# Ghostish/Open3DSOT

Hardware: NVIDIA H100
Metric: template-search pairs/sec, BAT-Car fwd+bwd (higher is better)
Workload: dtype f32

## Files before the change

open3dsot_b200/csrc/pwmlp_tc.cu:

```cuda
#include "common.cuh"
#include "lift.cuh"
#include "tc_ptx.cuh"
#include "../../include/o3d_b200.h"

namespace {

struct TcAct {
    const float* x; int ld; const float* scale; const float* shift; int relu;
    struct Coef { float4 s, t; bool on; };
    template <int R> struct Batch { float4 v[R]; };
    __device__ __forceinline__ Coef prep(int k, int K) const {
        Coef c;
        c.on = k < K;
        c.s = make_float4(1.f, 1.f, 1.f, 1.f);
        c.t = make_float4(0.f, 0.f, 0.f, 0.f);
        if (c.on && scale) { c.s = ld4g(scale + k); c.t = ld4g(shift + k); }
        return c;
    }
    template <int R>
    __device__ __forceinline__ void fetch(Batch<R>& b, int p0, int stride, int P, int k, int K) const {
        const int kk = k < K ? k : 0;
#pragma unroll
        for (int i = 0; i < R; ++i) {
            const int p = p0 + i * stride;
            b.v[i] = ld4g(x + (size_t)(p < P ? p : P - 1) * ld + kk);
        }
    }
    template <int R>
    __device__ __forceinline__ float4 finish(const Batch<R>& b, const Coef& c, int i, int p, int P) const {
        float4 v = b.v[i];
        if (!(c.on && p < P)) return make_float4(0.f, 0.f, 0.f, 0.f);
        if (scale) { v.x = fmaf(v.x, c.s.x, c.t.x); v.y = fmaf(v.y, c.s.y, c.t.y); v.z = fmaf(v.z, c.s.z, c.t.z); v.w = fmaf(v.w, c.s.w, c.t.w); }
        if (relu) { v.x = fmaxf(v.x, 0.f); v.y = fmaxf(v.y, 0.f); v.z = fmaxf(v.z, 0.f); v.w = fmaxf(v.w, 0.f); }
        return v;
    }
    __device__ __forceinline__ void prefetch_rows(int p0, int rows, int P) const {
        if (p0 < P) o3d_prefetch_l2(x + (size_t)p0 * ld, (size_t)min(rows, P - p0) * ld * sizeof(float));
    }
};

struct TcLift {
    LiftView lv; const float* scale; const float* shift; int relu;
    int la;
    struct Coef { float4 s, t, u0, u1, u2, u3; bool on; };
    template <int R> struct Batch { float4 v[R]; float4 sv[R]; int nrow[R]; int tag; };
    __device__ __forceinline__ Coef prep(int k, int K) const {
        Coef c;
        c.on = k < K;
        c.s = make_float4(1.f, 1.f, 1.f, 1.f);
        c.t = c.u0 = c.u1 = c.u2 = c.u3 = make_float4(0.f, 0.f, 0.f, 0.f);
        if (c.on && scale) { c.s = ld4g(scale + k); c.t = ld4g(shift + k); }
        if (c.on && lv.u) { c.u0 = ld4g(lv.u + k); c.u1 = ld4g(lv.u + lv.ldz + k); c.u2 = ld4g(lv.u + 2 * lv.ldz + k); c.u3 = ld4g(lv.u + 3 * lv.ldz + k); }
        return c;
    }
    template <int R>
    __device__ __forceinline__ void fetch(Batch<R>& b, int p0, int stride, int P, int k, int K) const {
        const int kk = k < K ? k : 0;
        if (lv.z) {
            int row[R];
            if (b.tag == p0 + 1) {
#pragma unroll
                for (int i = 0; i < R; ++i) row[i] = b.nrow[i];
            } else if (R == 4 && stride == 1 && (p0 & 3) == 0 && p0 + 3 < P) {
                const int4 r4 = __ldg(reinterpret_cast<const int4*>(lv.gidx + p0));
                row[0] = r4.x; row[R > 1 ? 1 : 0] = r4.y; row[R > 2 ? 2 : 0] = r4.z; row[R > 3 ? 3 : 0] = r4.w;
            } else {
#pragma unroll
                for (int i = 0; i < R; ++i) {
                    const int p = p0 + i * stride;
                    row[i] = __ldg(lv.gidx + (p < P ? p : P - 1));
                }
            }
#pragma unroll
            for (int i = 0; i < R; ++i) b.v[i] = ld4g(lv.z + (size_t)row[i] * lv.ldz + kk);
            if (la == 0) {
#pragma unroll
                for (int i = 0; i < R; ++i) b.nrow[i] = row[i];
                b.tag = p0 + 1;
            } else {
                const int pn = p0 + la;
#pragma unroll
                for (int i = 0; i < R; ++i) {
                    const int p = pn + i * stride;
                    b.nrow[i] = __ldg(lv.gidx + (p < P ? p : P - 1));
                }
                b.tag = pn + 1;
            }
        }
        if (lv.s) {
#pragma unroll
            for (int i = 0; i < R; ++i) {
                const int p = p0 + i * stride;
                b.sv[i] = ld4g(lv.s + (size_t)(p < P ? p : P - 1) * 4);
            }
        }
    }
    template <int R>
    __device__ __forceinline__ float4 finish(const Batch<R>& b, const Coef& c, int i, int p, int P) const {
        const float4 zero = make_float4(0.f, 0.f, 0.f, 0.f);
        if (!(c.on && p < P)) return zero;
        float4 v = lift_val4(lv.z ? b.v[i] : zero, lv.s ? b.sv[i] : zero, c.u0, c.u1, c.u2, c.u3);
        if (scale) { v.x = fmaf(v.x, c.s.x, c.t.x); v.y = fmaf(v.y, c.s.y, c.t.y); v.z = fmaf(v.z, c.s.z, c.t.z); v.w = fmaf(v.w, c.s.w, c.t.w); }
        if (relu) { v.x = fmaxf(v.x, 0.f); v.y = fmaxf(v.y, 0.f); v.z = fmaxf(v.z, 0.f); v.w = fmaxf(v.w, 0.f); }
        return v;
    }
    __device__ __forceinline__ void prefetch_rows(int p0, int rows, int P) const {
        if (p0 >= P) return;
        const size_t n = (size_t)min(rows, P - p0);
        if (lv.z) o3d_prefetch_l2(lv.gidx + p0, n * sizeof(int32_t));
        if (lv.s) o3d_prefetch_l2(lv.s + (size_t)p0 * 4, n * 16);
    }
};

struct TcDy {
    const float* g; int ldg; const float* y; int ldy; const float* a; const float* b; const float* cc;
    const float* dpool; const int32_t* sel; int S; int ldp;
    int sh;
    struct Coef { float4 a, b, c; bool on; };
    template <int R> struct Batch { float4 g[R]; float4 y[R]; bool shared; };
    __device__ __forceinline__ Coef prep(int k, int K) const {
        Coef c;
        c.on = k < K;
        c.a = make_float4(1.f, 1.f, 1.f, 1.f);
        c.b = c.c = make_float4(0.f, 0.f, 0.f, 0.f);
        if (c.on && a) { c.a = ld4g(a + k); c.b = ld4g(b + k); c.c = ld4g(cc + k); }
        return c;
    }
    template <int R>
    __device__ __forceinline__ void fetch(Batch<R>& bt, int p0, int stride, int P, int k, int K) const {
        const int kk = k < K ? k : 0;
        bt.shared = false;
        if (dpool) {
            const int pf = p0 < P ? p0 : P - 1;
            const int pe = p0 + (R - 1) * stride;
            const int pl = pe < P ? pe : P - 1;
            if (R >= 2 && (pf >> sh) == (pl >> sh)) {
                bt.shared = true;
                const size_t go = (size_t)(pf >> sh) * ldp + kk;
                bt.g[0] = ld4g(dpool + go);
                const int4 sl = __ldg(reinterpret_cast<const int4*>(sel + go));
                bt.g[R >= 2 ? 1 : 0] = make_float4(__int_as_float(sl.x), __int_as_float(sl.y), __int_as_float(sl.z), __int_as_float(sl.w));
            } else {
#pragma unroll
                for (int i = 0; i < R; ++i) {
                    const int p = p0 + i * stride, pp = p < P ? p : P - 1;
                    const int s = pp & (S - 1);
                    const size_t go = (size_t)(pp >> sh) * ldp + kk;
                    const int4 sl = __ldg(reinterpret_cast<const int4*>(sel + go));
                    const float4 d = ld4g(dpool + go);
                    bt.g[i] = make_float4(sl.x == s ? d.x : 0.f, sl.y == s ? d.y : 0.f, sl.z == s ? d.z : 0.f, sl.w == s ? d.w : 0.f);
                }
            }
        } else {
#pragma unroll
            for (int i = 0; i < R; ++i) {
                const int p = p0 + i * stride;
                bt.g[i] = ld4g(g + (size_t)(p < P ? p : P - 1) * ldg + kk);
            }
        }
#pragma unroll
        for (int i = 0; i < R; ++i) {
            const int p = p0 + i * stride;
            bt.y[i] = a ? ld4g(y + (size_t)(p < P ? p : P - 1) * ldy + kk) : make_float4(0.f, 0.f, 0.f, 0.f);
        }
    }
    template <int R>
    __device__ __forceinline__ float4 finish(const Batch<R>& bt, const Coef& c, int i, int p, int P) const {
        if (!(c.on && p < P)) return make_float4(0.f, 0.f, 0.f, 0.f);
        float4 v = bt.g[i];
        if (bt.shared) {
            const int s = p & (S - 1);
            const float4 d = bt.g[0], sl = bt.g[R >= 2 ? 1 : 0];
            v = make_float4(__float_as_int(sl.x) == s ? d.x : 0.f, __float_as_int(sl.y) == s ? d.y : 0.f,
                            __float_as_int(sl.z) == s ? d.z : 0.f, __float_as_int(sl.w) == s ? d.w : 0.f);
        }
        if (a) {
            const float4 yy = bt.y[i];
            v.x = fmaf(c.a.x, v.x, fmaf(c.c.x, yy.x, c.b.x)); v.y = fmaf(c.a.y, v.y, fmaf(c.c.y, yy.y, c.b.y));
            v.z = fmaf(c.a.z, v.z, fmaf(c.c.z, yy.z, c.b.z)); v.w = fmaf(c.a.w, v.w, fmaf(c.c.w, yy.w, c.b.w));
        }
        return v;
    }
    __device__ __forceinline__ void prefetch_rows(int p0, int rows, int P) const {
        if (p0 >= P) return;
        const size_t n = (size_t)min(rows, P - p0);
        if (!dpool) o3d_prefetch_l2(g + (size_t)p0 * ldg, n * ldg * sizeof(float));
        if (a) o3d_prefetch_l2(y + (size_t)p0 * ldy, n * ldy * sizeof(float));
        if (dpool) {
            const int g0 = p0 >> sh, g1 = (p0 + (int)n - 1) >> sh;
            const size_t bytes = (size_t)(g1 - g0 + 1) * ldp * sizeof(float);
            o3d_prefetch_l2(dpool + (size_t)g0 * ldp, bytes);
            o3d_prefetch_l2(sel + (size_t)g0 * ldp, bytes);
        }
    }
};

template <class L> struct Bf16 : L {};
template <class L> struct is_bf16 { static constexpr bool value = false; };
template <class L> struct is_bf16<Bf16<L>> { static constexpr bool value = true; };

template <int LD>
struct TcFwdEpi {
    float* y; int ldy; const float* bias; double* sum; double* sumsq;
    int S, log2S; float* ymax; float* ymin; int32_t* arg; int ldp;
    float bv, mx, mn; int ax, an; double d1, d2;
    __device__ __forceinline__ void begin(int ch, int Nw) {
        d1 = d2 = 0.0;
        bv = (bias && ch < Nw) ? bias[ch] : 0.f;
        mx = -INFINITY; mn = INFINITY; ax = an = 0;
    }
    __device__ __forceinline__ void prefetch(int, int, int, int) {}
    __device__ __forceinline__ const int32_t* lift_gidx() const { return nullptr; }
    __device__ __forceinline__ const float* lift_s() const { return nullptr; }
    __device__ __forceinline__ void set_tile(const int32_t*, const float4*) {}
    __device__ __forceinline__ void group(const uint32_t (&r)[16], int ch, int Nw, int pbase, int P) {
        if (ch >= Nw) return;
        float s1 = 0.f, s2 = 0.f;
        const int smask = S - 1;
        float* yp = y ? y + (size_t)pbase * ldy + ch : nullptr;
        if (pbase + 16 <= P && (S == 0 || S >= 16)) {
            float v[16];
#pragma unroll
            for (int j = 0; j < 16; ++j) v[j] = __uint_as_float(r[j]) + bv;
            if (yp) {
                const size_t st = LD ? (size_t)LD : (size_t)ldy;
#pragma unroll
                for (int j = 0; j < 16; ++j) yp[j * st] = v[j];
            }
#pragma unroll
            for (int j = 0; j < 16; ++j) {
                s1 += v[j];
                s2 = fmaf(v[j], v[j], s2);
            }
            if (S > 0) {
                float gm = v[0], gn = v[0];
                int ga = 0, gb = 0;
#pragma unroll
                for (int j = 1; j < 16; ++j) {
                    if (v[j] > gm) { gm = v[j]; ga = j; }
                    if (v[j] < gn) { gn = v[j]; gb = j; }
                }
                const int s0 = pbase & smask;
                if (s0 == 0) { mx = gm; ax = ga; mn = gn; an = gb; }
                else {
                    if (gm > mx) { mx = gm; ax = s0 + ga; }
                    if (gn < mn) { mn = gn; an = s0 + gb; }
                }
                if (s0 + 16 == S) {
                    const size_t o = (size_t)(pbase >> log2S) * ldp + ch;
                    ymax[o] = mx; ymin[o] = mn; arg[o] = ax | (an << 16);
                }
            }
        } else {
#pragma unroll
            for (int j = 0; j < 16; ++j) {
                if (pbase + j >= P) break;
                const float v = __uint_as_float(r[j]) + bv;
                if (yp) yp[(size_t)j * ldy] = v;
                s1 += v;
                s2 = fmaf(v, v, s2);
                if (S > 0) {
                    const int s = (pbase + j) & smask;
                    if (s == 0) { mx = -INFINITY; mn = INFINITY; ax = an = 0; }
                    if (v > mx) { mx = v; ax = s; }
                    if (v < mn) { mn = v; an = s; }
                    if (s == smask) {
                        const size_t o = (size_t)((pbase + j) >> log2S) * ldp + ch;
                        ymax[o] = mx; ymin[o] = mn; arg[o] = ax | (an << 16);
                    }
                }
            }
        }
        d1 += (double)s1;
        d2 += (double)s2;
    }
// ... 181 lines not shown
                                             kb == 0);
                }
                wgmma_commit();
                wgmma_wait<0>();
                wgmma_fence_acc(acc);
                if (lane == 0) o3d_mbar_arrive(empty + stage);
                if (++stage == TC_STAGES) { stage = 0; phase ^= 1; }
            }
            asm volatile("bar.sync %0, 128;" ::"r"(2 + h) : "memory");
            stage_acc(acc, stg, TC_EPI_LD);
            asm volatile("bar.sync %0, 128;" ::"r"(2 + h) : "memory");
            const float* row = stg + tw * TC_EPI_LD;
#pragma unroll 1
            for (int cg = 0; cg < 4; ++cg) {
                uint32_t r[16];
#pragma unroll
                for (int j = 0; j < 4; ++j) {
                    const float4 v = *reinterpret_cast<const float4*>(row + cg * 16 + 4 * j);
                    r[4 * j] = __float_as_uint(v.x); r[4 * j + 1] = __float_as_uint(v.y);
                    r[4 * j + 2] = __float_as_uint(v.z); r[4 * j + 3] = __float_as_uint(v.w);
                }
                epi.group(r, ch, Nw, pb + cg * 16, P);
                if (cg + 1 < 4) epi.prefetch(ch, Nw, pb + (cg + 1) * 16, P);
            }
            buf ^= 1;
        }
        epi.end(ch, Nw);
    } else {
        const int pt = (warp - 8) * 32 + lane;
        const int chunk = pt & 7;
        const int row0 = (pt >> 3) * 4;
        int stage = 0, phase = 0;
        struct Cur { int t, kb, p0; };
        auto advance = [&](Cur& c) {
            if (++c.kb == nkb) {
                c.kb = 0;
                c.t += gridDim.x;
                if (c.t < n_ptiles) c.p0 = tile_of(c.t) * TC_N;
            }
        };
        using Batch4 = typename BLoad::template Batch<4>;
        auto issue = [&](Batch4& r, typename BLoad::Coef& cf, const Cur& c) {
            if (c.t >= n_ptiles) return;
            const int k = c.kb * TC_K + chunk * 4;
            cf = bl.prep(k, K);
            bl.fetch(r, c.p0 + row0, 1, P, k, K);
        };
        Cur c0{(int)blockIdx.x, 0, 0};
        if (c0.t < n_ptiles) c0.p0 = tile_of(c0.t) * TC_N;
        Batch4 r0{};
        typename BLoad::Coef f0 = bl.prep(chunk * 4, K);
        issue(r0, f0, c0);
        if (pt == 0 && c0.t < n_ptiles) bl.prefetch_rows(c0.p0, TC_N, P);
        while (c0.t < n_ptiles) {
            o3d_mbar_wait(empty + stage, phase ^ 1);
            if (pt == 0) {
                o3d_mbar_expect_tx(full + stage, WBYTES);
                o3d_bulk_g2s(smem + stage * TC_STAGE_BYTES, wtiles + ((size_t)mt0 * nkb + c0.kb) * WBYTES, WBYTES, full + stage);
                const int tn = c0.t + (int)gridDim.x;
                if (c0.kb == 0 && tn < n_ptiles) bl.prefetch_rows(tile_of(tn) * TC_N, TC_N, P);
            }
            uint8_t* xhi = smem + stage * TC_STAGE_BYTES + 2 * TILE_BYTES;
            uint8_t* xlo = xhi + TILE_BYTES;
#pragma unroll
            for (int i = 0; i < 4; ++i) {
                const float4 v = bl.finish(r0, f0, i, c0.p0 + row0 + i, P);
                if constexpr (BF) {
                    *reinterpret_cast<uint2*>(xhi + sw64(row0 + i, chunk >> 1) + (chunk & 1) * 8) = pack_bf16x4(v);
                } else {
                    const uint32_t off = sw128(row0 + i, chunk);
                    *reinterpret_cast<float4*>(xhi + off) = hi_part(v);
                    *reinterpret_cast<float4*>(xlo + off) = lo_part(v);
                }
            }
            o3d_fence_proxy_async();
            o3d_mbar_arrive(full + stage);
            if (++stage == TC_STAGES) { stage = 0; phase ^= 1; }
            advance(c0);
            issue(r0, f0, c0);
        }
    }
}

constexpr int WG_STAGES = 3;
constexpr int WG_AHEAD = 4;
constexpr int WG_THREADS = 512;
constexpr int WG_SMEM = WG_STAGES * 4 * TILE_BYTES + 1024 + 256;

template <class L>
__device__ __forceinline__ void store_transposed(const L& ld, const typename L::template Batch<4>& raw, const typename L::Coef& cf,
                                                 uint8_t* hi, int c_local, int p_first, int prow0, int pend) {
#pragma unroll
    for (int i = 0; i < 4; ++i) {
        const int pl = prow0 + 8 * i;
        const float4 v = ld.finish(raw, cf, i, p_first + pl, pend);
        const float e[4] = {v.x, v.y, v.z, v.w};
#pragma unroll
        for (int j = 0; j < 4; ++j) {
            const uint32_t off = sw128(c_local + j, pl >> 2) + (uint32_t)((pl & 3) * 4);
            const float h = hi1(e[j]);
            *reinterpret_cast<float*>(hi + off) = h;
            *reinterpret_cast<float*>(hi + TILE_BYTES + off) = e[j] - h;
        }
    }
}

template <class XB>
__global__ void __launch_bounds__(WG_THREADS, 1)
    pw_wgrad_tc_kernel(TcDy da, XB xb, int P, int M, int N, int chunk, float* __restrict__ part) {
    extern __shared__ uint8_t smem_raw[];
    uint8_t* smem = reinterpret_cast<uint8_t*>((reinterpret_cast<uintptr_t>(smem_raw) + 1023) & ~(uintptr_t)1023);
    uint64_t* full = reinterpret_cast<uint64_t*>(smem + WG_STAGES * 4 * TILE_BYTES);
    uint64_t* empty = full + WG_STAGES;

    const int warp = threadIdx.x >> 5, lane = threadIdx.x & 31;
    const int m0 = blockIdx.z * TC_M, n0 = blockIdx.y * TC_N;
    const int pbeg = blockIdx.x * chunk, pend = min(P, pbeg + chunk);
    const int nkb = pend > pbeg ? (pend - pbeg + TC_K - 1) / TC_K : 0;
    auto kpos = [&](int i) { return pbeg + i * TC_K; };

    if (threadIdx.x == 0) {
        for (int s = 0; s < WG_STAGES; ++s) {
            o3d_mbar_init(full + s, 256);
            o3d_mbar_init(empty + s, 8);
        }
        o3d_fence_mbar_init();
    }
    __syncthreads();

    if (warp < 8) {
        const int h = warp >> 2, w = warp & 3;
        float acc[64];
#pragma unroll
        for (int i = 0; i < 64; ++i) acc[i] = 0.f;
        int stage = 0, phase = 0;
        for (int kb = 0; kb < nkb; ++kb) {
            o3d_mbar_wait(full + stage, phase);
            const uint32_t sb = o3d_smem_u32(smem + stage * 4 * TILE_BYTES);
            const uint32_t ab = sb + h * (TILE_BYTES / 2);
            wgmma_fence_acc(acc);
            wgmma_fence();
            wgmma_3xtf32_kblock<128>(acc, make_desc(ab), make_desc(ab + TILE_BYTES), make_desc(sb + 2 * TILE_BYTES),
                                     make_desc(sb + 3 * TILE_BYTES), kb == 0);
            wgmma_commit();
            wgmma_wait<0>();
            wgmma_fence_acc(acc);
            if (lane == 0) o3d_mbar_arrive(empty + stage);
            if (++stage == WG_STAGES) { stage = 0; phase ^= 1; }
        }
        const int Mt = TC_M * (int)gridDim.z, Nt = TC_N * (int)gridDim.y;
        float* __restrict__ out = part + (size_t)blockIdx.x * Mt * Nt;
#pragma unroll
        for (int i = 0; i < 64; i += 4) {
#pragma unroll
            for (int rr = 0; rr < 2; ++rr) {
                const int m = m0 + h * 64 + 16 * w + (lane >> 2) + 8 * rr, n = n0 + 8 * (i >> 2) + 2 * (lane & 3);
                *reinterpret_cast<float2*>(out + (size_t)m * Nt + n) = make_float2(acc[i + 2 * rr], acc[i + 2 * rr + 1]);
            }
        }
    } else {
        const int pw = warp - 8;
        const int c4 = pw * 4 + (lane & 3), prow0 = lane >> 2;
        const bool pt0 = pw == 0 && lane == 0;
        TcDy::Batch<4> ra = {};
        typename XB::template Batch<4> rb = {};
        auto fetch = [&](int kb) {
            da.fetch(ra, kpos(kb) + prow0, 8, pend, m0 + c4 * 4, M);
            xb.fetch(rb, kpos(kb) + prow0, 8, pend, n0 + c4 * 4, N);
        };
        auto prefetch = [&](int kb) {
            if (pt0 && kb < nkb) {
                da.prefetch_rows(kpos(kb), TC_K, pend);
                xb.prefetch_rows(kpos(kb), TC_K, pend);
            }
        };
        int stage = 0, phase = 0;
        for (int kb = 0; kb < WG_AHEAD; ++kb) prefetch(kb);
        if (nkb > 0) fetch(0);
        for (int kb = 0; kb < nkb; ++kb) {
            prefetch(kb + WG_AHEAD);
            o3d_mbar_wait(empty + stage, phase ^ 1);
            uint8_t* sbase = smem + stage * 4 * TILE_BYTES;
            store_transposed(da, ra, da.prep(m0 + c4 * 4, M), sbase, c4 * 4, kpos(kb), prow0, pend);
            store_transposed(xb, rb, xb.prep(n0 + c4 * 4, N), sbase + 2 * TILE_BYTES, c4 * 4, kpos(kb), prow0, pend);
            o3d_fence_proxy_async();
            o3d_mbar_arrive(full + stage);
            if (kb + 1 < nkb) fetch(kb + 1);
            if (++stage == WG_STAGES) { stage = 0; phase ^= 1; }
        }
    }
}

__global__ void __launch_bounds__(256)
    wgrad_reduce_kernel(const float* __restrict__ part, int splits, int Mt, int Nt, int M, int N, float* __restrict__ dW,
                        int lddw) {
    const int sub = threadIdx.x & 7;
    const int n4 = (blockIdx.x * 32 + (threadIdx.x >> 3)) * 4, m = blockIdx.y;
    float4 acc = make_float4(0.f, 0.f, 0.f, 0.f);
    if (n4 < N && m < M) {
        const float* p = part + (size_t)m * Nt + n4;
        for (int s = sub; s < splits; s += 8) {
            const float4 v = __ldg(reinterpret_cast<const float4*>(p + (size_t)s * Mt * Nt));
            acc.x += v.x; acc.y += v.y; acc.z += v.z; acc.w += v.w;
        }
    }
#pragma unroll
    for (int o = 4; o >= 1; o >>= 1) {
        acc.x += __shfl_xor_sync(0xFFFFFFFFu, acc.x, o); acc.y += __shfl_xor_sync(0xFFFFFFFFu, acc.y, o);
        acc.z += __shfl_xor_sync(0xFFFFFFFFu, acc.z, o); acc.w += __shfl_xor_sync(0xFFFFFFFFu, acc.w, o);
    }
    if (sub == 0 && n4 < N && m < M) {
        float* o = dW + (size_t)m * lddw + n4;
        o[0] += acc.x;
        if (n4 + 1 < N) o[1] += acc.y;
        if (n4 + 2 < N) o[2] += acc.z;
        if (n4 + 3 < N) o[3] += acc.w;
    }
}

__global__ void w_pretile_kernel(const float* __restrict__ W, int ld, int rows, int K, int nkb, uint8_t* __restrict__ out) {
    const int m_tile = blockIdx.y, kb = blockIdx.x;
    uint8_t* dst = out + ((size_t)m_tile * nkb + kb) * (2 * TILE_BYTES);
    for (int id = threadIdx.x; id < TC_M * 8; id += blockDim.x) {
        const int r = id >> 3, c = id & 7;
        const int row = m_tile * TC_M + r, k = kb * TC_K + c * 4;
        float4 v = make_float4(0.f, 0.f, 0.f, 0.f);
        if (row < rows && k < K) v = *reinterpret_cast<const float4*>(W + (size_t)row * ld + k);
        const uint32_t off = sw128(r, c);
        *reinterpret_cast<float4*>(dst + off) = hi_part(v);
        *reinterpret_cast<float4*>(dst + TILE_BYTES + off) = lo_part(v);
    }
}

inline int ilog2_exact(int v) { int l = 0; while ((1 << l) < v) ++l; return l; }

template <class BLoad, class Epi>
int launch_tc(BLoad bl, const uint8_t* wtiles, int P, int K, int Nw, Epi epi, bool reverse, cudaStream_t st, const char* name) {
    auto kern = pw_tc_kernel<BLoad, Epi>;
    O3D_CUDA(cudaFuncSetAttribute(kern, cudaFuncAttributeMaxDynamicSharedMemorySize, TC_SMEM), name);
    const int gy = (Nw + TC_M - 1) / TC_M;
    const int nkb = (K + TC_K - 1) / TC_K;
    const int n_ptiles = (P + TC_N - 1) / TC_N;
    int gx = o3d_num_sms() / gy;
    if (gx < 1) gx = 1;
    if (gx > n_ptiles) gx = n_ptiles;
    kern<<<dim3(gx, gy), TC_THREADS, TC_SMEM, st>>>(bl, wtiles, P, K, Nw, nkb, epi, reverse);
    O3D_CHECK_LAUNCH(name);
    return O3D_OK;
}

template <int LD, class BLoad>
int launch_fwd(const BLoad& bl, const void* wtiles, const float* bias, int P, int K, int Nw, float* y, int ldy, double* sum,
               double* sumsq, int S, float* ymax, float* ymin, int32_t* arg, int ldp, bool reverse, cudaStream_t st) {
    TcFwdEpi<LD> ep{};
    ep.y = y; ep.ldy = ldy; ep.bias = bias; ep.sum = sum; ep.sumsq = sumsq;
    ep.S = S; ep.ymax = ymax; ep.ymin = ymin; ep.arg = arg; ep.ldp = ldp;
    ep.log2S = 0;
    while ((1 << ep.log2S) < S) ++ep.log2S;
    return launch_tc(bl, (const uint8_t*)wtiles, P, K, Nw, ep, reverse, st, "o3d_pw_fwd_tc");
}

template <int LD, bool LIFT = false>
int launch_dgrad(const TcDy& bl, const void* wtiles_t, int P, int Cout, int Cin, float* out, int ldo, const float* yprev,
                 int ldyp, const float* pscale, const float* pshift, int prelu, double* s1, double* s2y, cudaStream_t st,
                 const LiftView* lv = nullptr) {
    if constexpr (!LIFT) {
        if (lv) return launch_dgrad<LD, true>(bl, wtiles_t, P, Cout, Cin, out, ldo, yprev, ldyp, pscale, pshift, prelu, s1, s2y, st, lv);
    }
    TcDgradEpi<LD, LIFT> ep{};
    if (lv) ep.lv = *lv;
    ep.out = out; ep.ldo = ldo; ep.yprev = yprev; ep.ldyp = ldyp; ep.scale = pscale; ep.shift = pshift; ep.relu = prelu;
    ep.s1g = s1; ep.s2y = s2y;
// ... 17 lines not shown
    return O3D_OK;
}

int o3d_pw_fwd_tc_dir(const float* x, int ldx, const float* in_scale, const float* in_shift, int in_relu, const void* wtiles,
                      const float* bias, int P, int K, int N, float* y, int ldy, double* sum, double* sumsq, int S, float* ymax,
                      float* ymin, int32_t* arg, int ldp, void* stream, bool reverse, bool bf16) {
    O3D_REQUIRE(x && wtiles, O3D_ERR_ARG, "o3d_pw_fwd_tc: null pointer");
    O3D_REQUIRE(P >= 0 && K >= 4 && N >= 1 && (K & 3) == 0 && (ldx & 3) == 0, O3D_ERR_ARG, "o3d_pw_fwd_tc: bad sizes");
    O3D_REQUIRE(S == 0 || (P % S == 0 && 64 % S == 0 && ymax && ymin && arg), O3D_ERR_ARG,
                "o3d_pw_fwd_tc: pooling group size must divide 64 and P");
    if (P == 0) return O3D_OK;
    const int Nw = (N + 3) & ~3;
    TcAct bl{x, ldx, in_scale, in_shift, in_relu};
    cudaStream_t st = (cudaStream_t)stream;
    if (bf16) {
        Bf16<TcAct> bb{bl};
#define O3D_FWD_ARGS bb, wtiles, bias, P, K, Nw, y, ldy, sum, sumsq, S, ymax, ymin, arg, ldp, reverse, st
        if (ldy == 64) return launch_fwd<64>(O3D_FWD_ARGS);
        if (ldy == 128) return launch_fwd<128>(O3D_FWD_ARGS);
        if (ldy == 256) return launch_fwd<256>(O3D_FWD_ARGS);
        return launch_fwd<0>(O3D_FWD_ARGS);
#undef O3D_FWD_ARGS
    }
#define O3D_FWD_ARGS bl, wtiles, bias, P, K, Nw, y, ldy, sum, sumsq, S, ymax, ymin, arg, ldp, reverse, st
    if (ldy == 64) return launch_fwd<64>(O3D_FWD_ARGS);
    if (ldy == 128) return launch_fwd<128>(O3D_FWD_ARGS);
    if (ldy == 256) return launch_fwd<256>(O3D_FWD_ARGS);
    return launch_fwd<0>(O3D_FWD_ARGS);
#undef O3D_FWD_ARGS
}

extern "C" int o3d_pw_fwd_tc(const float* x, int ldx, const float* in_scale, const float* in_shift, int in_relu,
                             const void* wtiles, const float* bias, int P, int K, int N, float* y, int ldy, double* sum,
                             double* sumsq, int S, float* ymax, float* ymin, int32_t* arg, int ldp, void* stream) {
    return o3d_pw_fwd_tc_dir(x, ldx, in_scale, in_shift, in_relu, wtiles, bias, P, K, N, y, ldy, sum, sumsq, S, ymax, ymin, arg,
                             ldp, stream, false, false);
}

namespace {
int dgrad_tc_impl(const float* g, int ldg, const float* y, int ldy, const float* a, const float* b, const float* cc,
                  const float* dpool, const int32_t* sel, int S, int ldp, const void* wtiles_t, int P, int Cout, int Cin,
                  float* out, int ldo, const float* yprev, int ldyp, const float* pscale, const float* pshift, int prelu,
                  double* s1, double* s2y, void* stream, const LiftView* lv) {
    O3D_REQUIRE((g || dpool) && wtiles_t && out, O3D_ERR_ARG, "o3d_pw_dgrad_tc: null pointer");
    O3D_REQUIRE((Cout & 3) == 0 && (Cin & 3) == 0, O3D_ERR_ARG, "o3d_pw_dgrad_tc: channel counts must be multiples of 4");
    if (P == 0) return O3D_OK;
    TcDy bl{g, ldg, y, ldy, a, b, cc, dpool, sel, S > 0 ? S : 1, ldp, ilog2_exact(S > 0 ? S : 1)};
    cudaStream_t st = (cudaStream_t)stream;
    const int ld = (!yprev || ldyp == ldo) ? ldo : 0;
#define O3D_DG_ARGS bl, wtiles_t, P, Cout, Cin, out, ldo, yprev, ldyp, pscale, pshift, prelu, s1, s2y, st, lv
    if (ld == 64) return launch_dgrad<64>(O3D_DG_ARGS);
    if (ld == 128) return launch_dgrad<128>(O3D_DG_ARGS);
    if (ld == 256) return launch_dgrad<256>(O3D_DG_ARGS);
    return launch_dgrad<0>(O3D_DG_ARGS);
#undef O3D_DG_ARGS
}
}

extern "C" int o3d_pw_dgrad_tc(const float* g, int ldg, const float* y, int ldy, const float* a, const float* b,
                               const float* cc, const float* dpool, const int32_t* sel, int S, int ldp,
                               const void* wtiles_t, int P, int Cout, int Cin, float* out, int ldo, const float* yprev,
                               int ldyp, const float* pscale, const float* pshift, int prelu, double* s1, double* s2y,
                               void* stream) {
    return dgrad_tc_impl(g, ldg, y, ldy, a, b, cc, dpool, sel, S, ldp, wtiles_t, P, Cout, Cin, out, ldo, yprev, ldyp, pscale,
                         pshift, prelu, s1, s2y, stream, nullptr);
}

extern "C" int o3d_pw_dgrad_tc_lift(const float* g, int ldg, const float* y, int ldy, const float* a, const float* b,
                                    const float* cc, const float* dpool, const int32_t* sel, int S, int ldp,
                                    const void* wtiles_t, int P, int Cout, int Cin, float* out, int ldo,
                                    const o3d_lift_t* lf, const int32_t* gidx, const float* pscale, const float* pshift,
                                    int prelu, double* s1, double* s2y, void* stream) {
    O3D_REQUIRE(lf && (gidx || !lf->z) && (lf->z || lf->s) && lf->ldz == Cin, O3D_ERR_ARG, "o3d_pw_dgrad_tc_lift: lift descriptor");
    const LiftView lv{lf->z, lf->ldz, lf->z ? gidx : nullptr, lf->s, lf->u};
    return dgrad_tc_impl(g, ldg, y, ldy, a, b, cc, dpool, sel, S, ldp, wtiles_t, P, Cout, Cin, out, ldo, nullptr, 0, pscale,
                         pshift, prelu, s1, s2y, stream, &lv);
}

namespace {
template <class XB>
int launch_wgrad(const TcDy& da, const XB& xb, int P, int Cout, int Cin, float* dw, int lddw, float* part, long long part_floats,
                 cudaStream_t st) {
    auto kern = pw_wgrad_tc_kernel<XB>;
    O3D_CUDA(cudaFuncSetAttribute(kern, cudaFuncAttributeMaxDynamicSharedMemorySize, WG_SMEM), "o3d_pw_wgrad_tc2");
    const int mt = (Cout + TC_M - 1) / TC_M, nt = (Cin + TC_N - 1) / TC_N;
    const int Mt = mt * TC_M, Nt = nt * TC_N;
    int splits = o3d_num_sms() / (mt * nt);
    if (splits < 1) splits = 1;
    const long long cap = part_floats / ((long long)Mt * Nt);
    if (splits > cap) splits = (int)cap;
    const int by_size = (P + 127) / 128;
    if (splits > by_size) splits = by_size;
    O3D_REQUIRE(splits >= 1, O3D_ERR_ARG, "o3d_pw_wgrad_tc2: workspace too small");
    int chunk = (P + splits - 1) / splits;
    chunk = ((chunk + TC_K - 1) / TC_K) * TC_K;
    splits = (P + chunk - 1) / chunk;
    kern<<<dim3(splits, nt, mt), WG_THREADS, WG_SMEM, st>>>(da, xb, P, Cout, Cin, chunk, part);
    O3D_CHECK_LAUNCH("o3d_pw_wgrad_tc2");
    dim3 rg((Cin / 4 + 31) / 32, Cout);
    wgrad_reduce_kernel<<<rg, 256, 0, st>>>(part, splits, Mt, Nt, Cout, Cin, dw, lddw);
    O3D_CHECK_LAUNCH("o3d_pw_wgrad_tc2: reduce");
    return O3D_OK;
}
inline TcLift make_tclift(const o3d_lift_t* lf, const int32_t* gidx, const float* scale, const float* shift, int relu) {
    return TcLift{LiftView{lf->z, lf->ldz, lf->z ? gidx : nullptr, lf->s, lf->u}, scale, shift, relu, 0};
}
}

extern "C" long long o3d_pw_wgrad_tc2_workspace_floats(void) {
    return (long long)o3d_num_sms() * TC_M * TC_N;
}

extern "C" int o3d_pw_wgrad_tc2(const float* g, int ldg, const float* y, int ldy, const float* a, const float* b,
                                const float* cc, const float* dpool, const int32_t* sel, int S, int ldp, const float* x,
                                int ldx, const float* in_scale, const float* in_shift, int in_relu, int P, int Cout,
                                int Cin, float* dw, int lddw, float* part, long long part_floats, void* stream) {
    O3D_REQUIRE((g || dpool) && x && dw && part, O3D_ERR_ARG, "o3d_pw_wgrad_tc2: null pointer");
    O3D_REQUIRE((Cout & 3) == 0 && (Cin & 3) == 0 && (ldx & 3) == 0 && (lddw & 3) == 0, O3D_ERR_ARG,
                "o3d_pw_wgrad_tc2: channel counts / leading dimensions must be multiples of 4");
    if (P == 0) return O3D_OK;
    TcDy da{g, ldg, y, ldy, a, b, cc, dpool, sel, S > 0 ? S : 1, ldp, ilog2_exact(S > 0 ? S : 1)};
    TcAct xb{x, ldx, in_scale, in_shift, in_relu};
    return launch_wgrad(da, xb, P, Cout, Cin, dw, lddw, part, part_floats, (cudaStream_t)stream);
}

extern "C" int o3d_pw_wgrad_tc_lift(const float* g, int ldg, const float* y, int ldy, const float* a, const float* b,
                                    const float* cc, const float* dpool, const int32_t* sel, int S, int ldp,
                                    const o3d_lift_t* lf, const int32_t* gidx, const float* in_scale, const float* in_shift,
                                    int in_relu, int P, int Cout, int Cin, float* dw, int lddw, float* part,
                                    long long part_floats, void* stream) {
    O3D_REQUIRE((g || dpool) && lf && (gidx || !lf->z) && dw && part, O3D_ERR_ARG, "o3d_pw_wgrad_tc_lift: null pointer");
    O3D_REQUIRE((Cout & 3) == 0 && (Cin & 3) == 0 && lf->ldz == Cin && (lddw & 3) == 0, O3D_ERR_ARG,
                "o3d_pw_wgrad_tc_lift: channel counts / leading dimensions");
    if (P == 0) return O3D_OK;
    TcDy da{g, ldg, y, ldy, a, b, cc, dpool, sel, S > 0 ? S : 1, ldp, ilog2_exact(S > 0 ? S : 1)};
    TcLift xb = make_tclift(lf, gidx, in_scale, in_shift, in_relu);
    xb.la = TC_K;
    return launch_wgrad(da, xb, P, Cout, Cin, dw, lddw, part, part_floats, (cudaStream_t)stream);
}

int o3d_pw_fwd_tc_lift_prec(const o3d_lift_t* lf, const int32_t* gidx, const float* in_scale, const float* in_shift, int in_relu,
                            const void* wtiles, const float* bias, int P, int K, int N, float* y, int ldy, double* sum,
                            double* sumsq, int S, float* ymax, float* ymin, int32_t* arg, int ldp, void* stream, bool bf16) {
    O3D_REQUIRE(lf && (gidx || !lf->z) && wtiles, O3D_ERR_ARG, "o3d_pw_fwd_tc_lift: null pointer");
    O3D_REQUIRE(P >= 0 && K >= 32 && N >= 1 && (K & 3) == 0 && lf->ldz == K, O3D_ERR_ARG, "o3d_pw_fwd_tc_lift: bad sizes");
    O3D_REQUIRE(S == 0 || (P % S == 0 && 64 % S == 0 && ymax && ymin && arg), O3D_ERR_ARG,
                "o3d_pw_fwd_tc_lift: pooling group size must divide 64 and P");
    if (P == 0) return O3D_OK;
    const int Nw = (N + 3) & ~3;
    const TcLift bl = make_tclift(lf, gidx, in_scale, in_shift, in_relu);
    cudaStream_t st = (cudaStream_t)stream;
    if (bf16) {
        const Bf16<TcLift> bb{bl};
#define O3D_FWD_ARGS bb, wtiles, bias, P, K, Nw, y, ldy, sum, sumsq, S, ymax, ymin, arg, ldp, false, st
        if (ldy == 64) return launch_fwd<64>(O3D_FWD_ARGS);
        if (ldy == 128) return launch_fwd<128>(O3D_FWD_ARGS);
        if (ldy == 256) return launch_fwd<256>(O3D_FWD_ARGS);
        return launch_fwd<0>(O3D_FWD_ARGS);
#undef O3D_FWD_ARGS
    }
#define O3D_FWD_ARGS bl, wtiles, bias, P, K, Nw, y, ldy, sum, sumsq, S, ymax, ymin, arg, ldp, false, st
    if (ldy == 64) return launch_fwd<64>(O3D_FWD_ARGS);
    if (ldy == 128) return launch_fwd<128>(O3D_FWD_ARGS);
    if (ldy == 256) return launch_fwd<256>(O3D_FWD_ARGS);
    return launch_fwd<0>(O3D_FWD_ARGS);
#undef O3D_FWD_ARGS
}

extern "C" int o3d_pw_fwd_tc_lift(const o3d_lift_t* lf, const int32_t* gidx, const float* in_scale, const float* in_shift,
                                  int in_relu, const void* wtiles, const float* bias, int P, int K, int N, float* y, int ldy,
                                  double* sum, double* sumsq, int S, float* ymax, float* ymin, int32_t* arg, int ldp,
                                  void* stream) {
    return o3d_pw_fwd_tc_lift_prec(lf, gidx, in_scale, in_shift, in_relu, wtiles, bias, P, K, N, y, ldy, sum, sumsq, S, ymax, ymin,
                                   arg, ldp, stream, false);
}
```

open3dsot_b200/csrc/tc_ptx.cuh:

```cuda
#pragma once
#include "common.cuh"

namespace {

constexpr int TC_M = 128;
constexpr int TC_N = 128;
constexpr int TC_K = 32;
constexpr int TILE_BYTES = TC_M * TC_K * 4;

__device__ __forceinline__ void wgmma_fence() { asm volatile("wgmma.fence.sync.aligned;" ::: "memory"); }
__device__ __forceinline__ void wgmma_commit() { asm volatile("wgmma.commit_group.sync.aligned;" ::: "memory"); }
template <int N>
__device__ __forceinline__ void wgmma_wait() { asm volatile("wgmma.wait_group.sync.aligned %0;" ::"n"(N) : "memory"); }
template <int R>
__device__ __forceinline__ void wgmma_fence_acc(float (&d)[R]) {
#pragma unroll
    for (int i = 0; i < R; ++i) asm volatile("" : "+f"(d[i])::"memory");
}

__device__ __forceinline__ void wgmma_tf32_n64(float (&d)[32], uint64_t adesc, uint64_t bdesc, uint32_t accumulate) {
    asm volatile(
        "{\n\t.reg .pred p;\n\t"
        "setp.ne.b32 p, %34, 0;\n\t"
        "wgmma.mma_async.sync.aligned.m64n64k8.f32.tf32.tf32 "
        "{%0, %1, %2, %3, %4, %5, %6, %7, %8, %9, %10, %11, %12, %13, %14, %15, %16, %17, %18, %19, %20, %21, %22, %23, %24, %25, %26, %27, %28, %29, %30, %31}, "
        "%32, %33, p, 1, 1;\n\t}"
        : "+f"(d[0]), "+f"(d[1]), "+f"(d[2]), "+f"(d[3]), "+f"(d[4]), "+f"(d[5]), "+f"(d[6]), "+f"(d[7]), "+f"(d[8]), "+f"(d[9]), "+f"(d[10]), "+f"(d[11]), "+f"(d[12]), "+f"(d[13]), "+f"(d[14]), "+f"(d[15]), "+f"(d[16]), "+f"(d[17]), "+f"(d[18]), "+f"(d[19]), "+f"(d[20]), "+f"(d[21]), "+f"(d[22]), "+f"(d[23]), "+f"(d[24]), "+f"(d[25]), "+f"(d[26]), "+f"(d[27]), "+f"(d[28]), "+f"(d[29]), "+f"(d[30]), "+f"(d[31])
        : "l"(adesc), "l"(bdesc), "r"(accumulate)
        : "memory");
}

__device__ __forceinline__ void wgmma_tf32_n128(float (&d)[64], uint64_t adesc, uint64_t bdesc, uint32_t accumulate) {
    asm volatile(
        "{\n\t.reg .pred p;\n\t"
        "setp.ne.b32 p, %66, 0;\n\t"
        "wgmma.mma_async.sync.aligned.m64n128k8.f32.tf32.tf32 "
        "{%0, %1, %2, %3, %4, %5, %6, %7, %8, %9, %10, %11, %12, %13, %14, %15, %16, %17, %18, %19, %20, %21, %22, %23, %24, %25, %26, %27, %28, %29, %30, %31, %32, %33, %34, %35, %36, %37, %38, %39, %40, %41, %42, %43, %44, %45, %46, %47, %48, %49, %50, %51, %52, %53, %54, %55, %56, %57, %58, %59, %60, %61, %62, %63}, "
        "%64, %65, p, 1, 1;\n\t}"
        : "+f"(d[0]), "+f"(d[1]), "+f"(d[2]), "+f"(d[3]), "+f"(d[4]), "+f"(d[5]), "+f"(d[6]), "+f"(d[7]), "+f"(d[8]), "+f"(d[9]), "+f"(d[10]), "+f"(d[11]), "+f"(d[12]), "+f"(d[13]), "+f"(d[14]), "+f"(d[15]), "+f"(d[16]), "+f"(d[17]), "+f"(d[18]), "+f"(d[19]), "+f"(d[20]), "+f"(d[21]), "+f"(d[22]), "+f"(d[23]), "+f"(d[24]), "+f"(d[25]), "+f"(d[26]), "+f"(d[27]), "+f"(d[28]), "+f"(d[29]), "+f"(d[30]), "+f"(d[31]), "+f"(d[32]), "+f"(d[33]), "+f"(d[34]), "+f"(d[35]), "+f"(d[36]), "+f"(d[37]), "+f"(d[38]), "+f"(d[39]), "+f"(d[40]), "+f"(d[41]), "+f"(d[42]), "+f"(d[43]), "+f"(d[44]), "+f"(d[45]), "+f"(d[46]), "+f"(d[47]), "+f"(d[48]), "+f"(d[49]), "+f"(d[50]), "+f"(d[51]), "+f"(d[52]), "+f"(d[53]), "+f"(d[54]), "+f"(d[55]), "+f"(d[56]), "+f"(d[57]), "+f"(d[58]), "+f"(d[59]), "+f"(d[60]), "+f"(d[61]), "+f"(d[62]), "+f"(d[63])
        : "l"(adesc), "l"(bdesc), "r"(accumulate)
        : "memory");
}


__device__ __forceinline__ uint64_t make_desc(uint32_t smem_addr) {
    uint64_t d = 0;
    d |= (uint64_t)((smem_addr >> 4) & 0x3FFF);
    d |= (uint64_t)1 << 16;
    d |= (uint64_t)(1024 >> 4) << 32;
    d |= (uint64_t)1 << 62;
    return d;
}

__device__ __host__ __forceinline__ uint32_t sw128(int r, int c) {
    return (uint32_t)((r >> 3) * 1024 + (r & 7) * 128 + ((c ^ (r & 7)) << 4));
}

__device__ __forceinline__ float hi1(float x) { return __uint_as_float(__float_as_uint(x) & 0xFFFFE000u); }
__device__ __forceinline__ float4 hi_part(const float4& v) { return make_float4(hi1(v.x), hi1(v.y), hi1(v.z), hi1(v.w)); }
__device__ __forceinline__ float4 lo_part(const float4& v) {
    return make_float4(v.x - hi1(v.x), v.y - hi1(v.y), v.z - hi1(v.z), v.w - hi1(v.w));
}
__device__ __forceinline__ float4 ld4g(const float* p) { return __ldg(reinterpret_cast<const float4*>(p)); }

template <int N>
__device__ __forceinline__ void wgmma_3xtf32_kblock(float (&d)[N / 2], uint64_t ahi, uint64_t alo, uint64_t bhi, uint64_t blo,
                                                    bool first) {
#pragma unroll
    for (int ks = 0; ks < TC_K / 8; ++ks) {
        const uint64_t adv = (uint64_t)((ks * 32) >> 4);
        if constexpr (N == 64) {
            wgmma_tf32_n64(d, alo + adv, bhi + adv, (first && ks == 0) ? 0u : 1u);
            wgmma_tf32_n64(d, ahi + adv, blo + adv, 1u);
            wgmma_tf32_n64(d, ahi + adv, bhi + adv, 1u);
        } else {
            wgmma_tf32_n128(d, alo + adv, bhi + adv, (first && ks == 0) ? 0u : 1u);
            wgmma_tf32_n128(d, ahi + adv, blo + adv, 1u);
            wgmma_tf32_n128(d, ahi + adv, bhi + adv, 1u);
        }
    }
}

constexpr int TC_BF_ROW = 64;
constexpr int BF_TILE_BYTES = TC_M * TC_BF_ROW;

__device__ __forceinline__ void wgmma_bf16_n64(float (&d)[32], uint64_t adesc, uint64_t bdesc, uint32_t accumulate) {
    asm volatile(
        "{\n\t.reg .pred p;\n\t"
        "setp.ne.b32 p, %34, 0;\n\t"
        "wgmma.mma_async.sync.aligned.m64n64k16.f32.bf16.bf16 "
        "{%0, %1, %2, %3, %4, %5, %6, %7, %8, %9, %10, %11, %12, %13, %14, %15, %16, %17, %18, %19, %20, %21, %22, %23, %24, %25, %26, %27, %28, %29, %30, %31}, "
        "%32, %33, p, 1, 1, 0, 0;\n\t}"
        : "+f"(d[0]), "+f"(d[1]), "+f"(d[2]), "+f"(d[3]), "+f"(d[4]), "+f"(d[5]), "+f"(d[6]), "+f"(d[7]), "+f"(d[8]), "+f"(d[9]), "+f"(d[10]), "+f"(d[11]), "+f"(d[12]), "+f"(d[13]), "+f"(d[14]), "+f"(d[15]), "+f"(d[16]), "+f"(d[17]), "+f"(d[18]), "+f"(d[19]), "+f"(d[20]), "+f"(d[21]), "+f"(d[22]), "+f"(d[23]), "+f"(d[24]), "+f"(d[25]), "+f"(d[26]), "+f"(d[27]), "+f"(d[28]), "+f"(d[29]), "+f"(d[30]), "+f"(d[31])
        : "l"(adesc), "l"(bdesc), "r"(accumulate)
        : "memory");
}

__device__ __forceinline__ void wgmma_bf16_n128(float (&d)[64], uint64_t adesc, uint64_t bdesc, uint32_t accumulate) {
    asm volatile(
        "{\n\t.reg .pred p;\n\t"
        "setp.ne.b32 p, %66, 0;\n\t"
        "wgmma.mma_async.sync.aligned.m64n128k16.f32.bf16.bf16 "
        "{%0, %1, %2, %3, %4, %5, %6, %7, %8, %9, %10, %11, %12, %13, %14, %15, %16, %17, %18, %19, %20, %21, %22, %23, %24, %25, %26, %27, %28, %29, %30, %31, %32, %33, %34, %35, %36, %37, %38, %39, %40, %41, %42, %43, %44, %45, %46, %47, %48, %49, %50, %51, %52, %53, %54, %55, %56, %57, %58, %59, %60, %61, %62, %63}, "
        "%64, %65, p, 1, 1, 0, 0;\n\t}"
        : "+f"(d[0]), "+f"(d[1]), "+f"(d[2]), "+f"(d[3]), "+f"(d[4]), "+f"(d[5]), "+f"(d[6]), "+f"(d[7]), "+f"(d[8]), "+f"(d[9]), "+f"(d[10]), "+f"(d[11]), "+f"(d[12]), "+f"(d[13]), "+f"(d[14]), "+f"(d[15]), "+f"(d[16]), "+f"(d[17]), "+f"(d[18]), "+f"(d[19]), "+f"(d[20]), "+f"(d[21]), "+f"(d[22]), "+f"(d[23]), "+f"(d[24]), "+f"(d[25]), "+f"(d[26]), "+f"(d[27]), "+f"(d[28]), "+f"(d[29]), "+f"(d[30]), "+f"(d[31]), "+f"(d[32]), "+f"(d[33]), "+f"(d[34]), "+f"(d[35]), "+f"(d[36]), "+f"(d[37]), "+f"(d[38]), "+f"(d[39]), "+f"(d[40]), "+f"(d[41]), "+f"(d[42]), "+f"(d[43]), "+f"(d[44]), "+f"(d[45]), "+f"(d[46]), "+f"(d[47]), "+f"(d[48]), "+f"(d[49]), "+f"(d[50]), "+f"(d[51]), "+f"(d[52]), "+f"(d[53]), "+f"(d[54]), "+f"(d[55]), "+f"(d[56]), "+f"(d[57]), "+f"(d[58]), "+f"(d[59]), "+f"(d[60]), "+f"(d[61]), "+f"(d[62]), "+f"(d[63])
        : "l"(adesc), "l"(bdesc), "r"(accumulate)
        : "memory");
}

__device__ __forceinline__ uint64_t make_desc_sw64(uint32_t smem_addr) {
    uint64_t d = 0;
    d |= (uint64_t)((smem_addr >> 4) & 0x3FFF);
    d |= (uint64_t)1 << 16;
    d |= (uint64_t)(512 >> 4) << 32;
    d |= (uint64_t)2 << 62;
    return d;
}

__device__ __host__ __forceinline__ uint32_t sw64(int r, int c) {
    return (uint32_t)(r * TC_BF_ROW + ((c ^ ((r >> 1) & 3)) << 4));
}

__device__ __forceinline__ uint32_t pack_bf16x2(float a, float b) {
    uint32_t r;
    asm("cvt.rn.bf16x2.f32 %0, %1, %2;" : "=r"(r) : "f"(b), "f"(a));
    return r;
}
__device__ __forceinline__ uint2 pack_bf16x4(const float4& v) { return make_uint2(pack_bf16x2(v.x, v.y), pack_bf16x2(v.z, v.w)); }

template <int N>
__device__ __forceinline__ void wgmma_bf16_kblock(float (&d)[N / 2], uint64_t a, uint64_t b, bool first) {
#pragma unroll
    for (int ks = 0; ks < 2; ++ks) {
        const uint64_t adv = (uint64_t)((ks * 32) >> 4);
        if constexpr (N == 64) wgmma_bf16_n64(d, a + adv, b + adv, (first && ks == 0) ? 0u : 1u);
        else wgmma_bf16_n128(d, a + adv, b + adv, (first && ks == 0) ? 0u : 1u);
    }
}

}
```

Before: 2841.

## Stage wgrad producer loads through cp.async raw buffers and skip padded MMA columns

Result: faster. 2890 (median of 6 runs) (+1.7%).

```diff
diff --git a/open3dsot_b200/csrc/pwmlp_tc.cu b/open3dsot_b200/csrc/pwmlp_tc.cu
--- a/open3dsot_b200/csrc/pwmlp_tc.cu
+++ b/open3dsot_b200/csrc/pwmlp_tc.cu
@@ -1,9 +1,20 @@
+#include <type_traits>
+
 #include "common.cuh"
 #include "lift.cuh"
 #include "tc_ptx.cuh"
 #include "../../include/o3d_b200.h"
 
 namespace {
+
+constexpr int RAW_SLOT = 256 * 16;
+__device__ __forceinline__ void cp_async16(uint32_t dst, const void* src) {
+    asm volatile("cp.async.cg.shared.global [%0], [%1], 16;" ::"r"(dst), "l"(src) : "memory");
+}
+__device__ __forceinline__ void cp_async_commit() { asm volatile("cp.async.commit_group;" ::: "memory"); }
+template <int N>
+__device__ __forceinline__ void cp_async_wait() { asm volatile("cp.async.wait_group %0;" ::"n"(N) : "memory"); }
+__device__ __forceinline__ float4 lds4(const uint8_t* p) { return *reinterpret_cast<const float4*>(p); }
 
 struct TcAct {
     const float* x; int ld; const float* scale; const float* shift; int relu;
@@ -109,6 +120,34 @@
         const size_t n = (size_t)min(rows, P - p0);
         if (lv.z) o3d_prefetch_l2(lv.gidx + p0, n * sizeof(int32_t));
         if (lv.s) o3d_prefetch_l2(lv.s + (size_t)p0 * 4, n * 16);
+    }
+    __device__ __forceinline__ void copy_rows(Batch<4>& b, uint32_t dst, int p0, int P, int k, int K) const {
+        const int kk = k < K ? k : 0;
+        if (lv.z) {
+            int row[4];
+            if (b.tag == p0 + 1) {
+#pragma unroll
+                for (int i = 0; i < 4; ++i) row[i] = b.nrow[i];
+            } else {
+#pragma unroll
+                for (int i = 0; i < 4; ++i) row[i] = __ldg(lv.gidx + min(p0 + i, P - 1));
+            }
+#pragma unroll
+            for (int i = 0; i < 4; ++i) cp_async16(dst + i * RAW_SLOT, lv.z + (size_t)row[i] * lv.ldz + kk);
+#pragma unroll
+            for (int i = 0; i < 4; ++i) b.nrow[i] = __ldg(lv.gidx + min(p0 + la + i, P - 1));
+            b.tag = p0 + la + 1;
+        }
+    }
+    __device__ __forceinline__ void load_scalars(Batch<4>& b, int p0, int P) const {
+        if (lv.s) {
+#pragma unroll
+            for (int i = 0; i < 4; ++i) b.sv[i] = ld4g(lv.s + (size_t)min(p0 + i, P - 1) * 4);
+        }
+    }
+    __device__ __forceinline__ void load_rows(Batch<4>& b, const uint8_t* src) const {
+#pragma unroll
+        for (int i = 0; i < 4; ++i) b.v[i] = lds4(src + i * RAW_SLOT);
     }
 };
 
@@ -191,6 +230,44 @@
             const size_t bytes = (size_t)(g1 - g0 + 1) * ldp * sizeof(float);
             o3d_prefetch_l2(dpool + (size_t)g0 * ldp, bytes);
             o3d_prefetch_l2(sel + (size_t)g0 * ldp, bytes);
+        }
+    }
+    __device__ __forceinline__ bool shared_group(int p0, int P) const {
+        return (min(p0, P - 1) >> sh) == (min(p0 + 3, P - 1) >> sh);
+    }
+    __device__ __forceinline__ void copy_rows(uint32_t dst, int p0, int P, int k, int K) const {
+        const int kk = k < K ? k : 0;
+        if (dpool) {
+            if (shared_group(p0, P)) {
+                const size_t go = (size_t)(min(p0, P - 1) >> sh) * ldp + kk;
+                cp_async16(dst, dpool + go);
+                cp_async16(dst + RAW_SLOT, sel + go);
+            } else {
+#pragma unroll
+                for (int i = 0; i < 4; ++i) {
+                    const int pp = min(p0 + i, P - 1), s = pp & (S - 1);
+                    const size_t go = (size_t)(pp >> sh) * ldp + kk;
+                    const int4 sl = __ldg(reinterpret_cast<const int4*>(sel + go));
+                    const float4 d = ld4g(dpool + go);
+                    asm volatile("st.shared.v4.f32 [%0], {%1, %2, %3, %4};" ::"r"(dst + i * RAW_SLOT), "f"(sl.x == s ? d.x : 0.f),
+                                 "f"(sl.y == s ? d.y : 0.f), "f"(sl.z == s ? d.z : 0.f), "f"(sl.w == s ? d.w : 0.f) : "memory");
+                }
+            }
+        } else {
+#pragma unroll
+            for (int i = 0; i < 4; ++i) cp_async16(dst + i * RAW_SLOT, g + (size_t)min(p0 + i, P - 1) * ldg + kk);
+        }
+        if (a) {
+#pragma unroll
+            for (int i = 0; i < 4; ++i) cp_async16(dst + (4 + i) * RAW_SLOT, y + (size_t)min(p0 + i, P - 1) * ldy + kk);
+        }
+    }
+    __device__ __forceinline__ void load_rows(Batch<4>& bt, const uint8_t* src, int p0, int P) const {
+        bt.shared = dpool && shared_group(p0, P);
+#pragma unroll
+        for (int i = 0; i < 4; ++i) {
+            bt.g[i] = lds4(src + i * RAW_SLOT);
+            bt.y[i] = a ? lds4(src + (4 + i) * RAW_SLOT) : make_float4(0.f, 0.f, 0.f, 0.f);
         }
     }
 };
@@ -538,10 +615,12 @@
     }
 }
 
-constexpr int WG_STAGES = 3;
 constexpr int WG_AHEAD = 4;
 constexpr int WG_THREADS = 512;
-constexpr int WG_SMEM = WG_STAGES * 4 * TILE_BYTES + 1024 + 256;
+constexpr int WG_RAW_BYTES = 12 * RAW_SLOT;
+template <class XB> constexpr bool wg_raw = std::is_same<XB, TcLift>::value;
+template <class XB> constexpr int wg_stages = wg_raw<XB> ? 2 : 3;
+template <class XB> constexpr int wg_smem = wg_stages<XB> * 4 * TILE_BYTES + (wg_raw<XB> ? 2 * WG_RAW_BYTES : 0) + 1024 + 256;
 
 template <class L>
 __device__ __forceinline__ void store_transposed(const L& ld, const typename L::template Batch<4>& raw, const typename L::Coef& cf,
@@ -561,12 +640,30 @@
     }
 }
 
+template <class L>
+__device__ __forceinline__ void store_transposed16(const L& ld, const typename L::template Batch<4>& raw, const typename L::Coef& cf,
+                                                   uint8_t* hi, int c_local, int pg, int p0, int pend) {
+    float4 v[4];
+#pragma unroll
+    for (int i = 0; i < 4; ++i) v[i] = ld.finish(raw, cf, i, p0 + i, pend);
+    const float4 t[4] = {make_float4(v[0].x, v[1].x, v[2].x, v[3].x), make_float4(v[0].y, v[1].y, v[2].y, v[3].y),
+                         make_float4(v[0].z, v[1].z, v[2].z, v[3].z), make_float4(v[0].w, v[1].w, v[2].w, v[3].w)};
+#pragma unroll
+    for (int j = 0; j < 4; ++j) {
+        const uint32_t off = sw128(c_local + j, pg);
+        *reinterpret_cast<float4*>(hi + off) = hi_part(t[j]);
+        *reinterpret_cast<float4*>(hi + TILE_BYTES + off) = lo_part(t[j]);
+    }
+}
+
 template <class XB>
 __global__ void __launch_bounds__(WG_THREADS, 1)
     pw_wgrad_tc_kernel(TcDy da, XB xb, int P, int M, int N, int chunk, float* __restrict__ part) {
+    constexpr int WG_STAGES = wg_stages<XB>;
     extern __shared__ uint8_t smem_raw[];
     uint8_t* smem = reinterpret_cast<uint8_t*>((reinterpret_cast<uintptr_t>(smem_raw) + 1023) & ~(uintptr_t)1023);
-    uint64_t* full = reinterpret_cast<uint64_t*>(smem + WG_STAGES * 4 * TILE_BYTES);
+    uint8_t* raw = smem + WG_STAGES * 4 * TILE_BYTES;
+    uint64_t* full = reinterpret_cast<uint64_t*>(raw + (wg_raw<XB> ? 2 * WG_RAW_BYTES : 0));
     uint64_t* empty = full + WG_STAGES;
 
     const int warp = threadIdx.x >> 5, lane = threadIdx.x & 31;
@@ -586,24 +683,37 @@
 
     if (warp < 8) {
         const int h = warp >> 2, w = warp & 3;
+        const int width = __shfl_sync(0xFFFFFFFFu, m0 + h * 64 >= M ? 0 : (n0 + 64 >= N ? 64 : 128), 0);
         float acc[64];
 #pragma unroll
         for (int i = 0; i < 64; ++i) acc[i] = 0.f;
-        int stage = 0, phase = 0;
-        for (int kb = 0; kb < nkb; ++kb) {
-            o3d_mbar_wait(full + stage, phase);
-            const uint32_t sb = o3d_smem_u32(smem + stage * 4 * TILE_BYTES);
-            const uint32_t ab = sb + h * (TILE_BYTES / 2);
-            wgmma_fence_acc(acc);
-            wgmma_fence();
-            wgmma_3xtf32_kblock<128>(acc, make_desc(ab), make_desc(ab + TILE_BYTES), make_desc(sb + 2 * TILE_BYTES),
-                                     make_desc(sb + 3 * TILE_BYTES), kb == 0);
-            wgmma_commit();
+        auto mainloop = [&](auto nw) {
+            constexpr int NW = decltype(nw)::value;
+            int stage = 0, phase = 0;
+            for (int kb = 0; kb < nkb; ++kb) {
+                o3d_mbar_wait(full + stage, phase);
+                if constexpr (NW == 0) {
+                    if (lane == 0) o3d_mbar_arrive(empty + stage);
+                } else {
+                    const uint32_t sb = o3d_smem_u32(smem + stage * 4 * TILE_BYTES);
+                    const uint32_t ab = sb + h * (TILE_BYTES / 2);
+                    wgmma_fence_acc(acc);
+                    wgmma_fence();
+                    wgmma_3xtf32_kblock<NW>(acc, make_desc(ab), make_desc(ab + TILE_BYTES), make_desc(sb + 2 * TILE_BYTES),
+                                            make_desc(sb + 3 * TILE_BYTES), kb == 0);
+                    wgmma_commit();
+                    wgmma_wait<1>();
+                    wgmma_fence_acc(acc);
+                    if (kb > 0 && lane == 0) o3d_mbar_arrive(empty + (stage == 0 ? WG_STAGES - 1 : stage - 1));
+                }
+                if (++stage == WG_STAGES) { stage = 0; phase ^= 1; }
+            }
             wgmma_wait<0>();
             wgmma_fence_acc(acc);
-            if (lane == 0) o3d_mbar_arrive(empty + stage);
-            if (++stage == WG_STAGES) { stage = 0; phase ^= 1; }
-        }
+        };
+        if (width == 128) mainloop(std::integral_constant<int, 128>{});
+        else if (width == 64) mainloop(std::integral_constant<int, 64>{});
+        else mainloop(std::integral_constant<int, 0>{});
         const int Mt = TC_M * (int)gridDim.z, Nt = TC_N * (int)gridDim.y;
         float* __restrict__ out = part + (size_t)blockIdx.x * Mt * Nt;
 #pragma unroll
@@ -614,7 +724,7 @@
                 *reinterpret_cast<float2*>(out + (size_t)m * Nt + n) = make_float2(acc[i + 2 * rr], acc[i + 2 * rr + 1]);
             }
         }
-    } else {
+    } else if constexpr (!wg_raw<XB>) {
         const int pw = warp - 8;
         const int c4 = pw * 4 + (lane & 3), prow0 = lane >> 2;
         const bool pt0 = pw == 0 && lane == 0;
@@ -644,6 +754,48 @@
             if (kb + 1 < nkb) fetch(kb + 1);
             if (++stage == WG_STAGES) { stage = 0; phase ^= 1; }
         }
+    } else {
+        const int pw = warp - 8, pg = lane & 7, c4 = pw * 4 + (lane >> 3), tp = threadIdx.x - 256;
+        const uint32_t raw_t = o3d_smem_u32(raw) + tp * 16;
+        TcDy::Batch<4> ra = {};
+        TcLift::Batch<4> rb = {};
+        auto copy = [&](int kb) {
+            const uint32_t dst = raw_t + (kb & 1) * WG_RAW_BYTES;
+            da.copy_rows(dst, kpos(kb) + 4 * pg, pend, m0 + c4 * 4, M);
+            xb.copy_rows(rb, dst + 8 * RAW_SLOT, kpos(kb) + 4 * pg, pend, n0 + c4 * 4, N);
+        };
+        auto prefetch = [&](int kb) {
+            if (tp == 0 && kb < nkb) {
+                da.prefetch_rows(kpos(kb), TC_K, pend);
+                xb.prefetch_rows(kpos(kb), TC_K, pend);
+            }
+        };
+        int stage = 0, phase = 0;
+        for (int kb = 0; kb < WG_AHEAD; ++kb) prefetch(kb);
+        if (nkb > 0) {
+            copy(0);
+            xb.load_scalars(rb, kpos(0) + 4 * pg, pend);
+        }
+        cp_async_commit();
+        for (int kb = 0; kb < nkb; ++kb) {
+            prefetch(kb + WG_AHEAD);
+            if (kb + 1 < nkb) copy(kb + 1);
+            cp_async_commit();
+            cp_async_wait<1>();
+            const uint8_t* src = raw + (kb & 1) * WG_RAW_BYTES + tp * 16;
+            const int p0 = kpos(kb) + 4 * pg;
+            da.load_rows(ra, src, p0, pend);
+            xb.load_rows(rb, src + 8 * RAW_SLOT);
+            o3d_mbar_wait(empty + stage, phase ^ 1);
+            uint8_t* sbase = smem + stage * 4 * TILE_BYTES;
+            store_transposed16(da, ra, da.prep(m0 + c4 * 4, M), sbase, c4 * 4, pg, p0, pend);
+            store_transposed16(xb, rb, xb.prep(n0 + c4 * 4, N), sbase + 2 * TILE_BYTES, c4 * 4, pg, p0, pend);
+            o3d_fence_proxy_async();
+            o3d_mbar_arrive(full + stage);
+            if (kb + 1 < nkb) xb.load_scalars(rb, p0 + TC_K, pend);
+            if (++stage == WG_STAGES) { stage = 0; phase ^= 1; }
+        }
+        cp_async_wait<0>();
     }
 }
 
@@ -827,7 +979,8 @@
 int launch_wgrad(const TcDy& da, const XB& xb, int P, int Cout, int Cin, float* dw, int lddw, float* part, long long part_floats,
                  cudaStream_t st) {
     auto kern = pw_wgrad_tc_kernel<XB>;
-    O3D_CUDA(cudaFuncSetAttribute(kern, cudaFuncAttributeMaxDynamicSharedMemorySize, WG_SMEM), "o3d_pw_wgrad_tc2");
+    constexpr int smem = wg_smem<XB>;
+    O3D_CUDA(cudaFuncSetAttribute(kern, cudaFuncAttributeMaxDynamicSharedMemorySize, smem), "o3d_pw_wgrad_tc2");
     const int mt = (Cout + TC_M - 1) / TC_M, nt = (Cin + TC_N - 1) / TC_N;
     const int Mt = mt * TC_M, Nt = nt * TC_N;
     int splits = o3d_num_sms() / (mt * nt);
@@ -840,7 +993,7 @@
     int chunk = (P + splits - 1) / splits;
     chunk = ((chunk + TC_K - 1) / TC_K) * TC_K;
     splits = (P + chunk - 1) / chunk;
-    kern<<<dim3(splits, nt, mt), WG_THREADS, WG_SMEM, st>>>(da, xb, P, Cout, Cin, chunk, part);
+    kern<<<dim3(splits, nt, mt), WG_THREADS, smem, st>>>(da, xb, P, Cout, Cin, chunk, part);
     O3D_CHECK_LAUNCH("o3d_pw_wgrad_tc2");
     dim3 rg((Cin / 4 + 31) / 32, Cout);
     wgrad_reduce_kernel<<<rg, 256, 0, st>>>(part, splits, Mt, Nt, Cout, Cin, dw, lddw);
diff --git a/open3dsot_b200/csrc/tc_ptx.cuh b/open3dsot_b200/csrc/tc_ptx.cuh
--- a/open3dsot_b200/csrc/tc_ptx.cuh
+++ b/open3dsot_b200/csrc/tc_ptx.cuh
@@ -18,7 +18,9 @@
     for (int i = 0; i < R; ++i) asm volatile("" : "+f"(d[i])::"memory");
 }
 
-__device__ __forceinline__ void wgmma_tf32_n64(float (&d)[32], uint64_t adesc, uint64_t bdesc, uint32_t accumulate) {
+template <int R>
+__device__ __forceinline__ void wgmma_tf32_n64(float (&d)[R], uint64_t adesc, uint64_t bdesc, uint32_t accumulate) {
+    static_assert(R >= 32, "n64 accumulator");
     asm volatile(
         "{\n\t.reg .pred p;\n\t"
         "setp.ne.b32 p, %34, 0;\n\t"
@@ -63,9 +65,10 @@
 }
 __device__ __forceinline__ float4 ld4g(const float* p) { return __ldg(reinterpret_cast<const float4*>(p)); }
 
-template <int N>
-__device__ __forceinline__ void wgmma_3xtf32_kblock(float (&d)[N / 2], uint64_t ahi, uint64_t alo, uint64_t bhi, uint64_t blo,
+template <int N, int R>
+__device__ __forceinline__ void wgmma_3xtf32_kblock(float (&d)[R], uint64_t ahi, uint64_t alo, uint64_t bhi, uint64_t blo,
                                                     bool first) {
+    static_assert(R >= N / 2, "accumulator narrower than the MMA");
 #pragma unroll
     for (int ks = 0; ks < TC_K / 8; ++ks) {
         const uint64_t adv = (uint64_t)((ks * 32) >> 4);
```
